# gengshan-y/ppr-diffphys

Hardware: AMD Instinct MI355X
Metric: env-steps/sec (fwd+adjoint), Laikago 12-DoF, batch=4096, 1/2/4/8 MI355X (higher is better)
Workload: dtype f32; 1 GPU; laikago, mixed mi-trot/mi-spin mocap targets, 4096 envs in total (4096 on rank 0) x 100 sim steps (4 frames), dt=5e-4, fwd+adjoint, batch split only (no collective); global_batch=4096, envs_per_gpu=4096, sim_steps=100, segment_lanes=16, nan_grads=0

## Files before the change

ppr-diffphys_amd/csrc/pd_device.h:

```cpp
#pragma once
#include "pd_math.h"

enum { PD_JOINT_REVOLUTE = 1, PD_JOINT_FIXED = 3, PD_JOINT_FREE = 4, PD_JOINT_COMPOUND = 5 };
enum { PD_JT_REVOLUTE = 1, PD_JT_COMPOUND = 2, PD_JT_FIXED = 4 };

#define PD_REC 17
#define PD_ADJ 13
#define PD_W6 7

struct PdDevModel {
  int nb, nq, nqd, nc, ntiles, max_children, max_depth;
  const int *jtype, *jparent, *qstart, *qdstart, *depth;
  const unsigned long long *children;
  const float *X_p, *X_c, *axis, *com;
  const float *lim_lo, *lim_hi, *lim_ke, *lim_kd;
  const float4 *pts;
  const unsigned char *pt_mat;
  const float4 *materials;
  const float4 *body_sphere;
  const float4 *tile_lo, *tile_hi;
  const int *tile_pack;
  const int2 *body_tiles;
  const int *small_tiles;
  unsigned long long big_bodies;
// ... 678 lines not shown
    float adj_q = 0.f;
    a_tgt[0] = 0.f; a_act[0] = 0.f; a_ke[0] = 0.f; a_kd[0] = 0.f;
    joint_force_adj(q, qd, tgt[0], ke[0], kd[0], lo, up, lke, lkd, adj_jf, adj_q, adj_qd, a_tgt[0], a_ke[0], a_kd[0], a_act[0]);
    adj_w_err += axis_p * adj_qd; adj_axis_p += j.w_err * adj_qd;
    const float adj_da = adj_q * dq_dda;
    adj_r_err.x += c.axis.x * adj_da; adj_r_err.y += c.axis.y * adj_da; adj_r_err.z += c.axis.z * adj_da;
    adj_r_err.w += adj_q * dq_dw;
    adj_qrot_q(j.q_p, c.axis, adj_q_p, adj_axis_p);
    adj_qrot_q(s.r, c.axis, adj_q_c, adj_axis_c);
  }
  if ((JT & PD_JT_COMPOUND) && (ALL || c.type == PD_JOINT_COMPOUND)) {
    const v3 ax[3] = {V3(1, 0, 0), P.ax1, P.ax2};
    v3 adj_f_raw = clamp3_pass(f_raw, adj_f, 1.0e4f);
    adj_x_err += adj_f_raw * ake; adj_v_err += adj_f_raw * akd;
    v3 adj_t_raw = clamp3_pass(P.t_raw, adj_t, 1.0e4f);
    float adj_ang[3] = {0.f, 0.f, 0.f};
    v3 adj_ax[3] = {V3(0, 0, 0), V3(0, 0, 0), V3(0, 0, 0)};
    qt adj_q_w = Q4(0, 0, 0, 0);
    const float *Mw = P.Mw;
    float aW[9];
#pragma unroll
    for (int k = 0; k < 9; ++k) aW[k] = 0.f;
#pragma unroll
    for (int k = 2; k >= 0; --k) {
      float adj_jf = dot(adj_t_raw, P.axw[k]);
      v3 adj_axw = adj_t_raw * P.jf[k];
      float adj_qdk = 0.f;
      a_tgt[k] = 0.f; a_act[k] = 0.f; a_ke[k] = 0.f; a_kd[k] = 0.f;
      const JointLimit L = c.lim[k];
      joint_force_adj(P.ang[k], P.qdk[k], tgt[k], ke[k], kd[k], L.lo, L.up, L.ke, L.kd, adj_jf, adj_ang[k], adj_qdk, a_tgt[k], a_ke[k],
                      a_kd[k], a_act[k]);
      adj_axw += j.w_err * adj_qdk; adj_w_err += P.axw[k] * adj_qdk;
      adj_ax[k] += matT_vec(Mw, adj_axw);
      add_outer(aW, adj_axw, ax[k]);
    }
    rotm_adj(P.q_w, aW, adj_q_w);
    if (HP) adj_q_p += adj_q_w; else adj_qmul_a(c.q_off, adj_q_p, adj_q_w);
    const float s0 = P.sc0.x, c0 = P.sc0.y;
    qt G;
    {
      const qt q = P.q10;
      const v3 g = adj_ax[2];
      G = Q4(g.x * (2.0f * q.z) - g.y * (2.0f * q.w), g.x * (2.0f * q.w) + g.y * (2.0f * q.z),
             g.x * (2.0f * q.x) + g.y * (2.0f * q.y) + g.z * (4.0f * q.z), g.x * (2.0f * q.y) - g.y * (2.0f * q.x) + g.z * (4.0f * q.w));
    }
    const qt adj_q_1 = Q4(c0 * G.x - s0 * G.w, c0 * G.y - s0 * G.z, c0 * G.z + s0 * G.y, c0 * G.w + s0 * G.x);
    float adj_q0x = P.q_1.w * G.x - P.q_1.y * G.z + P.q_1.z * G.y;
    float adj_q0w = P.q_1.w * G.w + P.q_1.y * G.y + P.q_1.z * G.z;
    adj_q_axis_angle_sc(ax[1], P.sc1.x, P.sc1.y, adj_ax[1], adj_ang[1], adj_q_1);
    adj_q0x += adj_ax[1].z * (2.0f * c0);
    adj_q0w += adj_ax[1].y * (4.0f * c0) + adj_ax[1].z * (2.0f * s0);
    adj_ang[0] += 0.5f * (c0 * adj_q0x - s0 * adj_q0w);
    qt adj_q_pc = Q4(0, 0, 0, 0);
    quat_decompose_adj(P.q_pc, P.c0, P.c1, P.c2, adj_ang, adj_q_pc);
    qt adj_qb = Q4(0, 0, 0, 0), adj_qa = adj_qb, adj_cqp = adj_qb;
    if (HP) adj_qb += adj_q_pc; else adj_qmul_a(c.q_off, adj_qb, adj_q_pc);
    adj_qmul(P.qa, s.r, adj_qa, adj_q_c, adj_qb);
    if (HP) adj_cqp += adj_qa; else adj_qmul_b(qconj(c.q_off), adj_cqp, adj_qa);
    adj_q_p += qconj(adj_cqp);
  }
  if (!((JT & PD_JT_COMPOUND) && (ALL || c.type == PD_JOINT_COMPOUND))) {
    qt adj_cqp = Q4(0, 0, 0, 0);
    adj_qmul(qconj(j.q_p), s.r, adj_cqp, adj_q_c, adj_r_err);
    adj_q_p += qconj(adj_cqp);
  }
  adj_qrot_q(s.r, c.com, adj_q_c, -adj_r_c);
  own.p += adj_x_err; own.r += adj_q_c; own.w += adj_w_err; own.v += adj_v_err;
  par = adj_zero();
  if (HP || c.parent >= 0) {
    v3 adj_x_p = adj_r_p - adj_x_err;
    par.p = adj_x_p - adj_r_p;
    float aP[9];
#pragma unroll
    for (int k = 0; k < 9; ++k) aP[k] = 0.f;
    add_outer(aP, -adj_r_p, c.com_par);
    add_outer(aP, adj_x_p, c.p_pj);
    rotm_adj(j.qp, aP, par.r);
    adj_qmul_a(c.q_pj, par.r, adj_q_p);
    par.w = -adj_w_err; par.v = -adj_v_err;
  }
}

#define PD_JC 23
#define PD_QPRE 22
#define PD_QGEN 3
struct RevCache {
  qt q_p, r_err;
  v3 x_p, axis_p, axis_c;
  float q, qd, jf, dq_dda, dq_dw;
};
PD_DEV void rev_cache_store(float *d, const RevCache &R) {
  d[0] = R.q_p.x; d[1] = R.q_p.y; d[2] = R.q_p.z; d[3] = R.q_p.w; d[4] = R.r_err.x; d[5] = R.r_err.y; d[6] = R.r_err.z; d[7] = R.r_err.w;
  d[8] = R.x_p.x; d[9] = R.x_p.y; d[10] = R.x_p.z;
  d[11] = R.axis_p.x; d[12] = R.axis_p.y; d[13] = R.axis_p.z; d[14] = R.axis_c.x; d[15] = R.axis_c.y; d[16] = R.axis_c.z;
  d[17] = R.q; d[18] = R.qd; d[19] = R.jf; d[20] = R.dq_dda; d[21] = R.dq_dw;
}
PD_DEV RevCache rev_cache_load(const float *d) {
  RevCache R;
  R.q_p = ld4(d); R.r_err = ld4(d + 4); R.x_p = ld3(d + 8); R.axis_p = ld3(d + 11); R.axis_c = ld3(d + 14);
  R.q = d[17]; R.qd = d[18]; R.jf = d[19]; R.dq_dda = d[20]; R.dq_dw = d[21];
  return R;
}

template <bool HP = false>
PD_DEV RevCache rev_forward(const PdDevModel &m, const BodyConst &c, qt q_c, v3 w_c, v3 pp, qt qp, v3 w_p, float tgt, float act, float ke,
                            float kd) {
  RevCache R;
  R.x_p = c.p_pj; R.q_p = c.q_pj;
  if (HP || c.parent >= 0) {
    R.x_p = pp + qrot(qp, c.p_pj);
    R.q_p = qmul(qp, c.q_pj);
  } else {
    w_p = V3(0, 0, 0);
  }
  R.r_err = qmul(qconj(R.q_p), q_c);
  R.axis_p = qrot(R.q_p, c.axis);
  R.axis_c = qrot(q_c, c.axis);
  R.q = twist_angle(dot(qvec(R.r_err), c.axis), R.r_err.w, c.alen, R.dq_dda, R.dq_dw);
  R.qd = dot(w_c - w_p, R.axis_p);
  const JointLimit L = c.lim[0];
  R.jf = joint_force(R.q, R.qd, tgt, ke, kd, act, L.lo, L.up, L.ke, L.kd);
  return R;
}

template <bool HP = false>
PD_DEV void rev_adjoint_core(const PdDevModel &m, const BodyConst &c, const BodyState &s, v3 rc_c, v3 pp, qt qp, v3 w_p, v3 v_p, v3 rc_par,
                             const RevCache &R, float tgt, float ke, float kd, v3 gc_t, v3 gc_f, v3 gp_t, v3 gp_f, BodyAdj &own, BodyAdj &par,
                             float *aR, float &a_tgt, float &a_act, float &a_ke, float &a_kd) {
  const float ake = m.attach_ke, akd = m.attach_kd, ads = 0.01f;
  v3 r_p = V3(0, 0, 0);
  if (HP || c.parent >= 0) {
    r_p = R.x_p - (pp + rc_par);
  } else {
    pp = V3(0, 0, 0); w_p = pp; v_p = pp; qp = Q4(0, 0, 0, 1);
  }
  const v3 r_c = s.p - (s.p + rc_c);
  const v3 x_err = s.p - R.x_p, v_err = s.v - v_p, w_err = s.w - w_p;
  const v3 f_total = x_err * ake + v_err * akd;
  v3 adj_t = -gc_t, adj_f = -gc_f, adj_r_c = V3(0, 0, 0), adj_r_p = V3(0, 0, 0);
  adj_cross(r_c, f_total, adj_r_c, adj_f, -gc_t);
  if (HP || c.parent >= 0) {
    adj_t += gp_t; adj_f += gp_f;
    adj_cross(r_p, f_total, adj_r_p, adj_f, gp_t);
  }
  v3 adj_x_err = adj_f * ake, adj_v_err = adj_f * akd, adj_w_err = adj_t * (akd * ads);
  qt adj_r_err = Q4(0, 0, 0, 0), adj_q_p = Q4(0, 0, 0, 0), adj_q_c = Q4(0, 0, 0, 0);
  const float adj_jf = dot(adj_t, R.axis_p);
  v3 adj_axis_p = adj_t * R.jf, adj_axis_c = V3(0, 0, 0);
  float adj_qd = -adj_jf * (akd * ads);
  adj_axis_p += adj_t * (-R.qd * (akd * ads));
  adj_cross(R.axis_p, R.axis_c, adj_axis_p, adj_axis_c, adj_t * ake);
  float adj_q = 0.f;
  a_tgt = 0.f; a_act = 0.f; a_ke = 0.f; a_kd = 0.f;
  const JointLimit L = c.lim[0];
  joint_force_adj(R.q, R.qd, tgt, ke, kd, L.lo, L.up, L.ke, L.kd, adj_jf, adj_q, adj_qd, a_tgt, a_ke, a_kd, a_act);
  adj_w_err += R.axis_p * adj_qd; adj_axis_p += w_err * adj_qd;
  const float adj_da = adj_q * R.dq_dda;
  adj_r_err.x += c.axis.x * adj_da; adj_r_err.y += c.axis.y * adj_da; adj_r_err.z += c.axis.z * adj_da;
  adj_r_err.w += adj_q * R.dq_dw;
  adj_qrot_q(R.q_p, c.axis, adj_q_p, adj_axis_p);
  add_outer(aR, adj_axis_c, c.axis);
  {
    qt adj_cqp = Q4(0, 0, 0, 0);
    adj_qmul(qconj(R.q_p), s.r, adj_cqp, adj_q_c, adj_r_err);
    adj_q_p += qconj(adj_cqp);
  }
// ... 130 lines not shown
```

ppr-diffphys_amd/csrc/pd_kernels.hip:

```cpp
#include "pd_device.h"
#include "pd_args.h"
#include "pd_se3.h"
#include "pd_quad.h"

#if PD_POLICY == 1
#define k_rollout_fwd k_rollout_fwd_literal
#define k_rollout_bwd k_rollout_bwd_literal
#define k_rollout_bwd3 k_rollout_bwd3_literal
#define PD_LAUNCH_NAME(w) PD_CAT(PD_CAT(pd_launch_seg, w), _literal)
#define PD_SET_LDS_NAME(w) PD_CAT(PD_CAT(pd_set_lds_seg, w), _literal)
#else
#define PD_LAUNCH_NAME(w) PD_CAT(pd_launch_seg, w)
#define PD_SET_LDS_NAME(w) PD_CAT(pd_set_lds_seg, w)
#endif

#ifdef PD_STAMPS
#define STAMP_DECL unsigned long long st_acc[16] = {0, 0, 0, 0, 0, 0, 0, 0, 0, 0, 0, 0, 0, 0, 0, 0}, st_t = pd_memtime()
#define STAMP_ARGS , unsigned long long *st_acc, unsigned long long &st_t
#define STAMP_PASS , st_acc, st_t
#define STAMP(i) do { unsigned long long t2_ = pd_memtime(); st_acc[i] += t2_ - st_t; st_t = t2_; } while (0)
#define STAMP_COUNT(i, n) do { st_acc[i] += (unsigned long long)(n); } while (0)
#define STAMP_FLUSH(a) do { if ((a).dbg && (threadIdx.x & 63) == 0) for (int i_ = 0; i_ < 16; ++i_) (a).dbg[((size_t)blockIdx.x * (blockDim.x / 64) + (threadIdx.x >> 6)) * 16 + i_] = st_acc[i_]; } while (0)
__device__ __forceinline__ unsigned long long pd_memtime() {
  unsigned long long t;
// ... 1242 lines not shown
template <int SEGW, int JT, bool QUAD = false, bool SEL = false>
__global__ __launch_bounds__(PD_BLOCK) void k_rollout_bwd(PdDevModel m, RolloutArgs a) {
  static_assert(JT == PD_JT_REVOLUTE, "the wave-specialised adjoint of revolute-only plain models: every jointed body is a revolute joint on a parent body");
  extern __shared__ __attribute__((aligned(16))) unsigned char smem[];
  constexpr int EPW = Seg<SEGW>::EPW;
  const int bw = (int)blockDim.x / (QUAD ? 192 : 128);
  const int role = (int)(threadIdx.x >> 6) / bw;
  const bool contact_wave = role != 0;
  [[maybe_unused]] const int knock_role = role;
  const int lane = threadIdx.x & 63, wave = (int)(threadIdx.x >> 6) % bw;
  const int seg = lane / SEGW, l = lane % SEGW;
  const int env = (blockIdx.x * bw + wave) * EPW + seg;
  const bool env_ok = env < a.bs;
  const int ec = env_ok ? env : 0;
  const bool is_body = env_ok && l < m.nb;
  const int b = l < m.nb ? l : m.nb - 1;
  const int nb = m.nb, N = a.bs * nb;

  SweepTables tabs;
  const int env_stride = m.env_lds_floats + 2 * m.env_lds_jc + (QUAD ? m.env_lds_rec2 : 0);
  float *scratch = lds_setup<false>(m, smem, tabs, wave * EPW + seg, env_stride);
  float4 *cull = (float4 *)scratch;
  float *rec = scratch + 4 * nb, *adjf = rec + nb * PD_REC, *cslot = adjf + nb * PD_W6, *cacc = cslot + (nb + 1) * PD_ADJ;
  int *list = (int *)(cacc + nb * PD_ADJ), *hits = list + m.list_cap;
  float *slot = (float *)(hits + PD_HIT_CAP_TILES * SEGW);
  float *jc = scratch + m.env_lds_floats;
  int *sig = (int *)(scratch - (size_t)seg * env_stride + m.env_lds_floats - 4);
  if (lane == 0 && !contact_wave) { sig[0] = 0; sig[1] = 0; sig[2] = 0; sig[3] = 0; }
  __syncthreads();
  PD_KNOCK_EXIT(false, knock_role);
  if constexpr (QUAD) {
    if (!env_ok) return;
  }

  BodyConst c = load_body_const(m, b, ec);
#pragma unroll
  for (int u = 0; u < 4; ++u) c.small_e[u] = m.small_tiles[u * 64 + (l < 64 ? l : 0)];
  if (l == 0) {
#pragma unroll
    for (int k = 0; k < PD_ADJ; ++k) cslot[nb * PD_ADJ + k] = 0.f;
  }
  int cz[4];
#pragma unroll
  for (int k = 0; k < 4; ++k) cz[k] = is_body && c.child[k] >= 0 ? c.child[k] : nb;
  const float *rec_s = rec;
  const float4 *cull_s = cull;
  auto contact_hit = [&](const float *r, float4 P, float4 mat, float *out) {
    const int pb = (int)(r - rec_s) / PD_REC;
    BodyAdj o = adj_zero();
    if constexpr (QUAD) {
      ContactPre C = contact_point_adj_pre(r, cull_s[pb], P, mat);
      contact_pre_barrier(C);
      contact_point_adj_rest(C, P, mat, ld3(adjf + pb * PD_W6), ld3(adjf + pb * PD_W6 + 3), o);
    } else {
      contact_point_adj(r, cull_s[pb], P, mat, ld3(adjf + pb * PD_W6), ld3(adjf + pb * PD_W6 + 3), o);
    }
    adj_store(out, o);
  };
  if (contact_wave) {
    STAMP_DECL;
    const bool rev = is_body && c.type == PD_JOINT_REVOLUTE;
    const size_t qd_off = (size_t)ec * m.nqd + c.qdstart;
    const float ke1 = rev ? a.target_ke[qd_off] : 0.f, kd1 = rev ? a.target_kd[qd_off] : 0.f;
    const int lq = l < PD_HITLOG - 1 ? l : PD_HITLOG - 2;
    const unsigned boff_c = (unsigned)((size_t)ec * nb + b) * 4u, boff_p = (unsigned)((size_t)ec * nb + (c.parent >= 0 ? c.parent : b)) * 4u;
    const unsigned boff_qd = (unsigned)qd_off * 4u, boff_lg = (unsigned)ec * (PD_HITLOG * 4u);
    auto load_log = [&](int step, int &cnt, int &e) {
      const int *lg = a.hitlog + (size_t)__builtin_amdgcn_readfirstlane(step > 0 ? step : 0) * a.bs * PD_HITLOG;
      cnt = __float_as_int(ldg((const float *)lg, boff_lg)); e = __float_as_int(ldg((const float *)lg + 1, boff_lg + (unsigned)lq * 4u));
    };
    auto load_ctrl = [&](int step, float &tgt, float &act) {
      const size_t o = (size_t)__builtin_amdgcn_readfirstlane(step > 0 ? step : 0) * a.bs * m.nqd;
      tgt = rev ? ldg(a.refs + o, boff_qd) : 0.f; act = rev && ptr_given<SEL>(a.torques) ? ldg(a.torques + o, boff_qd) : 0.f;
    };
    auto fetch_point = [&](int cnt, int &e, float4 &P, float4 &M) {
      if (!(env_ok && l < cnt && l < PD_HITLOG - 1)) e = 0;
      P = m.pts[e & 0xffff]; M = m.materials[(e >> 16) & 0xff];
    };
    auto load_pose = [&](int step, float4 *o) {
      const float *tj = a.ws + (size_t)__builtin_amdgcn_readfirstlane(step > 0 ? step : 0) * (PD_TRAJ_G * 4) * N;
      if (rev) {
        o[0] = ldg4(tj, boff_c * 4u); o[1] = ldg4(tj + (size_t)4 * N, boff_c * 4u);
        o[2] = ldg4(tj, boff_p * 4u); o[3] = ldg4(tj + (size_t)4 * N, boff_p * 4u); o[4] = ldg4(tj + (size_t)8 * N, boff_p * 4u);
      }
    };
    int cnt_c = 0, e_c = 0, cnt_n = 0, e_n = 0;
    float4 P_c, M_c;
    float tgt_c = 0.f, act_c = 0.f;
    float4 pose[5];
#pragma unroll
    for (int k = 0; k < 5; ++k) pose[k] = make_float4(0.f, 0.f, 0.f, 0.f);
    const int qb = lane >> 2, qc = lane & 3, bbq = qb < nb ? qb : nb - 1;
    const QLane kq = q_lane(qc);
    const int qgen_floats = m.env_lds_rec2 / PD_QGEN - PD_QPRE * 64 - m.env_lds_jc;
    float *const qgen = jc + 2 * m.env_lds_jc, *const qpre = qgen + PD_QGEN * qgen_floats;
    QBody Bq;
    float npl_c[PD_TRAJ_G];
    const unsigned boff_tjq = (unsigned)(((size_t)ec * nb + bbq) * 4 + qc) * 4u;
    auto load_planes = [&](int step, float *pl) {
      const float *tj = a.ws + (size_t)__builtin_amdgcn_readfirstlane(step > 0 ? step : 0) * (PD_TRAJ_G * 4) * N;
#pragma unroll
      for (int g = 0; g < PD_TRAJ_G; ++g) pl[g] = ldg(tj + (size_t)(4 * g) * N, boff_tjq);
    };
    auto q_pre = [&](const float *pl, int g) {
      QState s;
      const float vx = Q_BC3(pl[1]), vy = Q_BC3(pl[2]), vz = Q_BC0(pl[3]);
      const float tsh = q_dpp<PD_QP(1, 2, 3, 3)>(pl[3]);
      const float maskf = Q_BC3(pl[4]);
      s.r = pl[0];
      s.w = kq.isv ? pl[1] : 0.f; s.p = kq.isv ? pl[2] : 0.f;
      s.v = qc == 0 ? vx : (qc == 1 ? vy : (qc == 2 ? vz : 0.f));
      const float t0 = kq.isv ? tsh : 0.f, f0 = kq.isv ? pl[4] : 0.f;
      QM3 Rr, Rc;
      q_rotm(kq, s.r, Rr, Rc);
      const float rc = q_mvc(Rr, Bq.com0, Bq.com1, Bq.com2);
      {
        float *G = qgen + g * qgen_floats, *r = G + 4 * nb + bbq * PD_REC;
        r[3 + qc] = s.r;
        r[kq.isv ? qc : 16] = s.p; r[kq.isv ? 7 + qc : 16] = s.w; r[kq.isv ? 10 + qc : 16] = s.v; r[kq.isv ? 13 + qc : 16] = rc;
        if (qc == 1) ((float4 *)G)[bbq] = make_float4(s.p, Rr.a, Rr.b, Rr.c);
      }
      QIntTmp T;
      q_integrate_adj_pre(kq, Bq, s, Rr, Rc, t0, a.dt, T);
      float *P = qpre + g * (PD_QPRE * 64) + lane;
      P[0 * 64] = s.p; P[1 * 64] = s.r; P[2 * 64] = s.w; P[3 * 64] = s.v; P[4 * 64] = t0; P[5 * 64] = f0; P[6 * 64] = maskf; P[7 * 64] = rc;
      P[8 * 64] = Rr.a; P[9 * 64] = Rr.b; P[10 * 64] = Rr.c; P[11 * 64] = Rc.a; P[12 * 64] = Rc.b; P[13 * 64] = Rc.c;
      P[14 * 64] = T.wb; P[15 * 64] = T.Iwb; P[16 * 64] = T.tb; P[17 * 64] = T.u; P[18 * 64] = T.w1; P[19 * 64] = T.il; P[20 * 64] = T.r1;
    };
    int g3 = a.nsteps > 0 ? (a.nsteps - 1) % PD_QGEN : 0;
    if constexpr (QUAD) {
      if (role == 2) {
        const BodyConst cb = load_body_const(m, bbq, ec);
        const size_t qidx = (size_t)ec * nb + bbq;
        const int qv = qc < 3 ? qc : 2;
        Bq.com0 = cb.com.x; Bq.com1 = cb.com.y; Bq.com2 = cb.com.z;
        const float *Ib = a.inertia + qidx * 9, *Jb = a.inv_inertia + qidx * 9;
        Bq.I.a = kq.isv ? Ib[qv * 3] : 0.f; Bq.I.b = kq.isv ? Ib[qv * 3 + 1] : 0.f; Bq.I.c = kq.isv ? Ib[qv * 3 + 2] : 0.f;
        Bq.invI.a = kq.isv ? Jb[qv * 3] : 0.f; Bq.invI.b = kq.isv ? Jb[qv * 3 + 1] : 0.f; Bq.invI.c = kq.isv ? Jb[qv * 3 + 2] : 0.f;
        float *const jcq = qpre + PD_QGEN * (PD_QPRE * 64);
        if (a.nsteps > 0) { load_ctrl(a.nsteps - 1, tgt_c, act_c); load_pose(a.nsteps - 1, pose); load_planes(a.nsteps - 1, npl_c); }
        for (int step = a.nsteps - 1; step >= 0; --step) {
          PD_WAIT_VMEM();
          pair_wait(sig, a.nsteps - step - (PD_QGEN - 1));
          if (rev) {
            const qt q_c = Q4(pose[0].x, pose[0].y, pose[0].z, pose[0].w), qp = Q4(pose[2].x, pose[2].y, pose[2].z, pose[2].w);
            const v3 w_c = V3(pose[1].x, pose[1].y, pose[1].z), pp = V3(pose[4].x, pose[4].y, pose[4].z), w_p = V3(pose[3].x, pose[3].y, pose[3].z);
            rev_cache_store(jcq + g3 * m.env_lds_jc + b * PD_JC, rev_forward<true>(m, c, q_c, w_c, pp, qp, w_p, tgt_c, act_c, ke1, kd1));
          }
          q_pre(npl_c, g3);
          load_ctrl(step - 1, tgt_c, act_c); load_pose(step - 1, pose); load_planes(step - 1, npl_c);
          pair_signal(sig + 1, a.nsteps - step);
          g3 = g3 == 0 ? PD_QGEN - 1 : g3 - 1;
        }
        return;
      }
    }
    if (a.nsteps > 0) {
      load_log(a.nsteps - 1, cnt_c, e_c);
      if constexpr (!QUAD) { load_ctrl(a.nsteps - 1, tgt_c, act_c); load_pose(a.nsteps - 1, pose); }
      load_log(a.nsteps - 2, cnt_n, e_n);
      fetch_point(cnt_c, e_c, P_c, M_c);
    }
    for (int step = a.nsteps - 1; step >= 0; --step) {
      PD_WAIT_VMEM();
      if (!QUAD && rev)
      {
        const qt q_c = Q4(pose[0].x, pose[0].y, pose[0].z, pose[0].w), qp = Q4(pose[2].x, pose[2].y, pose[2].z, pose[2].w);
        const v3 w_c = V3(pose[1].x, pose[1].y, pose[1].z), pp = V3(pose[4].x, pose[4].y, pose[4].z), w_p = V3(pose[3].x, pose[3].y, pose[3].z);
        float *dst = jc + (step & 1) * m.env_lds_jc + b * PD_JC;
        rev_cache_store(dst, rev_forward<true>(m, c, q_c, w_c, pp, qp, w_p, tgt_c, act_c, ke1, kd1));
      }
      STAMP(8);
      float tgt_n, act_n;
      float4 P_n, M_n;
      int cnt_n2, e_n2;
      fetch_point(cnt_n, e_n, P_n, M_n);
      if constexpr (!QUAD) {
        load_ctrl(step - 1, tgt_n, act_n);
        load_pose(step - 1, pose);
      } else {
        tgt_n = 0.f; act_n = 0.f;
      }
      load_log(step - 2, cnt_n2, e_n2);
      const bool fast = __ballot(env_ok && (cnt_c < 0 || cnt_c > SEGW)) == 0ull;
      const int nh = fast && env_ok ? cnt_c : 0;
      STAMP(7);
      if constexpr (!QUAD) pair_signal(sig + 1, a.nsteps - step);
      const int pb = l < nh ? (e_c >> 24) & 0x3f : -2;
      ContactPre cpre;
      cpre.touch = false;
      if constexpr (QUAD) {
        pair_wait(sig + 1, a.nsteps - step);
        rec_s = qgen + g3 * qgen_floats + 4 * nb;
        cull_s = (const float4 *)(qgen + g3 * qgen_floats);
        if (fast && l < nh) cpre = contact_point_adj_pre(rec_s + pb * PD_REC, cull_s[pb], P_c, M_c);
      }
      pair_wait(sig, a.nsteps - step);
      __builtin_amdgcn_s_setprio(PD_PRIO_CRITICAL);
      STAMP(9);
      if (fast) {
        float out[PD_ADJ];
#pragma unroll
        for (int i = 0; i < PD_ADJ; ++i) out[i] = 0.f;
        if constexpr (QUAD) {
          if (l < nh) {
            BodyAdj o = adj_zero();
            contact_pre_barrier(cpre);
            contact_point_adj_rest(cpre, P_c, M_c, ld3(adjf + pb * PD_W6), ld3(adjf + pb * PD_W6 + 3), o);
            adj_store(out, o);
          }
        } else {
          if (l < nh) contact_hit(rec_s + pb * PD_REC, P_c, M_c, out);
        }
        STAMP(10);
        bool last;
        seg_run_sum<PD_ADJ>(out, pb, l, nh, last);
        if (last) {
#pragma unroll
          for (int i = 0; i < PD_ADJ; ++i) cacc[pb * PD_ADJ + i] = out[i];
        }
        STAMP(11);
      } else {
        float4 cv = make_float4(0.f, 0.f, 1.f, 0.f);
        if (is_body) cv = cull_s[b];
        int *lg = a.hitlog + ((size_t)step * a.bs + ec) * PD_HITLOG;
        const bool replay = __ballot(env_ok && cnt_c < 0) == 0ull;
        int log_n_unused;
        sweep_contacts<SEGW, PD_ADJ, PD_ADJ, false>(m, tabs, c, cv, rec_s, cull_s, list, hits, slot, cacc, is_body, env_ok, seg, l,
                                                    replay ? lg : nullptr, replay ? (env_ok ? cnt_c : 0) : PD_NO_REPLAY, log_n_unused,
                                                    contact_hit STAMP_PASS);
      }
      STAMP(12);
      pair_signal(sig + 2, a.nsteps - step);
      __builtin_amdgcn_s_setprio(0);
      cnt_c = cnt_n; e_c = e_n; P_c = P_n; M_c = M_n; tgt_c = tgt_n; act_c = act_n;
      cnt_n = cnt_n2; e_n = e_n2;
      if constexpr (QUAD) g3 = g3 == 0 ? PD_QGEN - 1 : g3 - 1;
    }
    STAMP_FLUSH(a);
    return;
  }
  if constexpr (QUAD) {
    static_assert(SEGW == 64, "quad-lane body wave: one env per wave");
    const int qb = lane >> 2, qc = lane & 3, bb = qb < nb ? qb : nb - 1, qv = qc < 3 ? qc : 2;
    const bool qbody = true;
    float *const dummy = adjf + bb * PD_W6 + 6;
    const QLane k = q_lane(qc);
    const size_t qidx = (size_t)ec * nb + bb;
    QBody B;
    QM3 It, invIt;
    float com_par0, com_par1, com_par2, p_pj0, p_pj1, p_pj2;
    QPerm pjc;
    {
      const BodyConst cb = load_body_const(m, bb, ec);
      B.type = cb.type; B.pidx = cb.pidx; B.qdstart = cb.qdstart;
      B.joint = qbody && cb.type == PD_JOINT_REVOLUTE;
      B.com = q_pick(k, cb.com); B.com0 = cb.com.x; B.com1 = cb.com.y; B.com2 = cb.com.z;
      B.axis = q_pick(k, cb.axis); B.ax0 = cb.axis.x; B.ax1 = cb.axis.y; B.ax2 = cb.axis.z; B.alen = cb.alen;
      B.p_pj = q_pick(k, cb.p_pj); B.q_pj = q_pick(k, cb.q_pj); B.pj = q_perm(k, B.q_pj);
      pjc = q_perm(k, B.q_pj * k.sc);
      com_par0 = cb.com_par.x; com_par1 = cb.com_par.y; com_par2 = cb.com_par.z;
      p_pj0 = cb.p_pj.x; p_pj1 = cb.p_pj.y; p_pj2 = cb.p_pj.z;
      B.g = q_pick(k, V3(m.gx, m.gy, m.gz));
      B.reach = cb.reach; B.sphere_w = cb.sphere.w; B.lim = cb.lim[0];
      B.inv_m = a.inv_mass[qidx];
      const bool on = cb.type == PD_JOINT_REVOLUTE;
      B.ke = on ? a.target_ke[(size_t)ec * m.nqd + cb.qdstart] : 0.f;
      B.kd = on ? a.target_kd[(size_t)ec * m.nqd + cb.qdstart] : 0.f;
      const float *Ib = a.inertia + qidx * 9, *Jb = a.inv_inertia + qidx * 9;
      B.I.a = k.isv ? Ib[qv * 3] : 0.f; B.I.b = k.isv ? Ib[qv * 3 + 1] : 0.f; B.I.c = k.isv ? Ib[qv * 3 + 2] : 0.f;
      B.invI.a = k.isv ? Jb[qv * 3] : 0.f; B.invI.b = k.isv ? Jb[qv * 3 + 1] : 0.f; B.invI.c = k.isv ? Jb[qv * 3 + 2] : 0.f;
      It.a = k.isv ? Ib[qv] : 0.f; It.b = k.isv ? Ib[3 + qv] : 0.f; It.c = k.isv ? Ib[6 + qv] : 0.f;
      invIt.a = k.isv ? Jb[qv] : 0.f; invIt.b = k.isv ? Jb[3 + qv] : 0.f; invIt.c = k.isv ? Jb[6 + qv] : 0.f;
    }
    int qcz[4];
    const unsigned long long q_children = m.children[bb];
#pragma unroll
    for (int j = 0; j < 4; ++j) { const int cid = (int)((q_children >> (8 * j)) & 0xffull); qcz[j] = (qbody && cid != 0xff) ? cid : nb; }
    if (lane < PD_ADJ) cslot[nb * PD_ADJ + lane] = 0.f;
    float *const ca_r = cacc + bb * PD_ADJ + 3 + qc, *const ca_p = k.isv ? cacc + bb * PD_ADJ + qc : dummy,
                *const ca_w = k.isv ? cacc + bb * PD_ADJ + 7 + qc : dummy, *const ca_v = k.isv ? cacc + bb * PD_ADJ + 10 + qc : dummy;
    float *const cs_r = cslot + bb * PD_ADJ + 3 + qc, *const cs_p = k.isv ? cslot + bb * PD_ADJ + qc : dummy,
                *const cs_w = k.isv ? cslot + bb * PD_ADJ + 7 + qc : dummy, *const cs_v = k.isv ? cslot + bb * PD_ADJ + 10 + qc : dummy;
    *ca_r = 0.f; *ca_p = 0.f; *ca_w = 0.f; *ca_v = 0.f;
    QM3 g_I, g_invI;
    g_I.a = g_I.b = g_I.c = 0.f; g_invI = g_I;
    float g_inv_m = 0.f, g_ke = 0.f, g_kd = 0.f;
    QAdj gn;
    gn.p = gn.r = gn.w = gn.v = 0.f;
    const unsigned boff_tj = (unsigned)(qidx * 4 + qc) * 4u, boff_qd = (unsigned)((size_t)ec * m.nqd + B.qdstart) * 4u;
    const unsigned boff_rf = (unsigned)(qidx * 6 + qv) * 4u;
    float n_tgt = 0.f;
    int n_fr = -1;
    auto load_step = [&](int step) {
      const int sc = __builtin_amdgcn_readfirstlane(step >= 0 ? step : 0);
      n_fr = a.frame_of_step[sc + 1];
      const size_t o = (size_t)sc * a.bs * m.nqd;
      n_tgt = ldg(a.refs + o, boff_qd);
    };
    const float ake = m.attach_ke, akd = m.attach_kd;
    const int qgen_floats = m.env_lds_rec2 / PD_QGEN - PD_QPRE * 64 - m.env_lds_jc;
    float *const qgen = jc + 2 * m.env_lds_jc, *const qpre = qgen + PD_QGEN * qgen_floats;
    QState s;
    float t0 = 0.f, f0 = 0.f, tgt = 0.f, rc = 0.f, sd_p = 0.f, sd_r = 0.f, sd_w = 0.f, sd_v = 0.f;
    unsigned mask = 0u;
    QM3 Rr, Rc;
    QIntTmp T;
    auto q_ahead = [&](int step) {
      const int fr = n_fr;
      sd_p = 0.f; sd_r = 0.f; sd_w = 0.f; sd_v = 0.f;
      if (fr >= 0) {
        const float *gp = a.adj_pos + ((size_t)fr * N + qidx) * 7, *gv = a.adj_vel + ((size_t)fr * N + qidx) * 6;
        sd_p = gp[qv]; sd_r = gp[3 + qc]; sd_w = gv[qv]; sd_v = gv[3 + qv];
      }
      tgt = n_tgt;
      load_step(step - 1);
    };
    auto q_take = [&](int g) {
      const float *P = qpre + g * (PD_QPRE * 64) + lane;
      s.p = P[0 * 64]; s.r = P[1 * 64]; s.w = P[2 * 64]; s.v = P[3 * 64]; t0 = P[4 * 64]; f0 = P[5 * 64]; mask = __float_as_uint(P[6 * 64]); rc = P[7 * 64];
// ... 112 lines not shown
    auto q_seeds = [&](int fr) {
      const float *gp = a.adj_pos + ((size_t)fr * N + qidx) * 7, *gv = a.adj_vel + ((size_t)fr * N + qidx) * 6;
      const float sp = gp[qv], sr = gp[3 + qc], sw = gv[qv], sv = gv[3 + qv];
      gn.p += k.isv ? sp : 0.f; gn.r += sr; gn.w += k.isv ? sw : 0.f; gn.v += k.isv ? sv : 0.f;
    };
    if (a.frame_of_step[0] >= 0) q_seeds(a.frame_of_step[0]);
    float *const rec0 = qgen + 4 * nb;
    WAVE_SYNC();
    if (qbody) {
      float *d = a.g_state0 ? a.g_state0 + qidx * PD_ADJ : cacc + bb * PD_ADJ;
      d[3 + qc] = gn.r;
      if (k.isv) { d[qc] = gn.p; d[7 + qc] = gn.w; d[10 + qc] = gn.v; }
    }
    WAVE_SYNC();
    if (!a.g_state0) {
      BodyAdj gs = adj_zero();
      if (is_body) adj_add_from(gs, cacc + b * PD_ADJ);
      if (a.nsteps == 0) {
        for (int d = 0; d <= m.max_depth; ++d) {
          if (is_body && c.depth == d) {
            BodyState s0 = fk_joint<JT>(c, a.q_init + (size_t)ec * m.nq + c.qstart, a.qd_init + (size_t)ec * m.nqd + c.qdstart, rec0);
            stage_record(rec0, b, s0, c.com);
          }
          WAVE_SYNC();
        }
      }
      for (int d = m.max_depth; d >= 0; --d) {
        if (is_body && c.depth == d) {
          for (int j = 0; j < m.max_children; ++j) {
            int cid = (int)((c.children >> (8 * j)) & 0xffull);
            if (cid != 0xff) adj_add_from(gs, cslot + cid * PD_ADJ);
          }
          BodyAdj pr_ = fk_joint_adj<JT, 1>(c, a.q_init + (size_t)ec * m.nq + c.qstart, a.qd_init + (size_t)ec * m.nqd + c.qdstart, rec0,
                                          gs, a.g_q_init + (size_t)ec * m.nq + c.qstart, a.g_qd_init + (size_t)ec * m.nqd + c.qdstart);
          adj_store(cslot + b * PD_ADJ, pr_);
        }
        WAVE_SYNC();
      }
    }
    if (qbody) {
      if (qc == 0) a.g_inv_mass[qidx] = NZ(g_inv_m);
      if (k.isv) {
        float *gi = a.g_inertia + qidx * 9 + qc * 3, *gj = a.g_inv_inertia + qidx * 9 + qc * 3;
        gi[0] = NZ(g_I.a); gi[1] = NZ(g_I.b); gi[2] = NZ(g_I.c);
        gj[0] = NZ(g_invI.a); gj[1] = NZ(g_invI.b); gj[2] = NZ(g_invI.c);
      }
      const size_t og = (size_t)ec * m.nqd + B.qdstart;
      if (B.type == PD_JOINT_REVOLUTE && qc == 0) { a.g_ke[og] = NZ(g_ke); a.g_kd[og] = NZ(g_kd); }
      if (B.type == PD_JOINT_FREE) {
        a.g_ke[og + qc] = 0.f; a.g_kd[og + qc] = 0.f;
        if (qc < 2) { a.g_ke[og + 4 + qc] = 0.f; a.g_kd[og + 4 + qc] = 0.f; }
      }
    }
    return;
  }
  constexpr int ND = 1;
  const size_t idx = (size_t)ec * nb + b;
  const int ndof = c.type == PD_JOINT_REVOLUTE ? 1 : (c.type == PD_JOINT_COMPOUND ? 3 : 0);

  float inv_m = a.inv_mass[idx], I[9], invI[9], ke[ND], kd[ND];
#pragma unroll
  for (int k = 0; k < 9; ++k) { I[k] = a.inertia[idx * 9 + k]; invI[k] = a.inv_inertia[idx * 9 + k]; }
#pragma unroll
  for (int k = 0; k < ND; ++k) {
    bool on = k < ndof;
    ke[k] = on ? a.target_ke[(size_t)ec * m.nqd + c.qdstart + k] : 0.f;
    kd[k] = on ? a.target_kd[(size_t)ec * m.nqd + c.qdstart + k] : 0.f;
  }
  float g_inv_m = 0.f, g_I[9], g_invI[9], g_ke[ND], g_kd[ND];
#pragma unroll
  for (int k = 0; k < 9; ++k) { g_I[k] = 0.f; g_invI[k] = 0.f; }
#pragma unroll
  for (int k = 0; k < ND; ++k) { g_ke[k] = 0.f; g_kd[k] = 0.f; }
  if (is_body) {
#pragma unroll
    for (int k = 0; k < PD_ADJ; ++k) cacc[b * PD_ADJ + k] = 0.f;
  }

  BodyAdj gn = adj_zero();
  BodyState s;
  s.p = V3(0, 0, 0); s.r = Q4(0, 0, 0, 1); s.w = V3(0, 0, 0); s.v = V3(0, 0, 0);

  const unsigned boff = (unsigned)idx * 4u, boff_qd = (unsigned)((size_t)ec * m.nqd + c.qdstart) * 4u;
  const bool zero_by_lanes = m.jtype[0] == PD_JOINT_FREE && nb >= 7;
  const unsigned boff_zero = (unsigned)((size_t)ec * m.nqd + m.qdstart[0] + (b >= 1 && b <= 6 ? b - 1 : 0)) * 4u;
  float4 n_s[PD_TRAJ_G];
  float n_tgt[ND];
  int n_fr = -1;
  auto load_step = [&](int step) {
    const int sc = __builtin_amdgcn_readfirstlane(step >= 0 ? step : 0);
    n_fr = a.frame_of_step[sc + 1];
    const float *tj = a.ws + (size_t)sc * (PD_TRAJ_G * 4) * N;
#pragma unroll
    for (int g = 0; g < PD_TRAJ_G; ++g) n_s[g] = ldg4(tj + (size_t)(4 * g) * N, boff * 4u);
    const size_t o = (size_t)sc * a.bs * m.nqd;
#pragma unroll
    for (int k = 0; k < ND; ++k) {
      bool on = k < ndof;
      n_tgt[k] = on ? ldg(a.refs + o + k, boff_qd) : 0.f;
    }
  };
  if (a.nsteps > 0) load_step(a.nsteps - 1);
  STAMP_DECL;
  for (int step = a.nsteps - 1; step >= 0; --step) {
    PD_WAIT_VMEM();
    {
      const int fr = n_fr;
      if (fr >= 0) {
        add_frame_seeds(a, fr, N, idx, gn);
      }
    }
    s.r = Q4(n_s[0].x, n_s[0].y, n_s[0].z, n_s[0].w); s.w = V3(n_s[1].x, n_s[1].y, n_s[1].z);
    s.p = V3(n_s[2].x, n_s[2].y, n_s[2].z); s.v = V3(n_s[1].w, n_s[2].w, n_s[3].x);
    v3 t0 = V3(n_s[3].y, n_s[3].z, n_s[3].w), f0 = V3(n_s[4].x, n_s[4].y, n_s[4].z);
    const unsigned clamp_mask = __float_as_uint(n_s[4].w);
    float tgt[ND];
#pragma unroll
    for (int k = 0; k < ND; ++k) tgt[k] = n_tgt[k];
    const size_t oc = (size_t)step * a.bs * m.nqd;
    load_step(step - 1);
    float Rm[9];
    rotm(s.r, Rm);
    const v3 rc = mat_vec(Rm, c.com);
    if (is_body) stage_record(rec, cull, b, s, rc, Rm);
    STAMP(0);
    BodyAdj ga = adj_zero();
    v3 adj_t0 = V3(0, 0, 0), adj_f0 = adj_t0;
    float aR[9];
#pragma unroll
    for (int k = 0; k < 9; ++k) aR[k] = 0.f;
    integrate_adj(m, c, s, Rm, clamp_mask, t0, f0, inv_m, I, invI, a.dt, gn, ga, aR, adj_t0, adj_f0, g_inv_m, g_I, g_invI);
    if (is_body) {
      float *f = adjf + b * PD_W6;
      f[0] = adj_t0.x; f[1] = adj_t0.y; f[2] = adj_t0.z; f[3] = adj_f0.x; f[4] = adj_f0.y; f[5] = adj_f0.z;
    }
    STAMP(1);
    pair_signal(sig, a.nsteps - step);
    if (grad_wanted<SEL>(a.g_res_f) && is_body) {
      float *o = a.g_res_f + (size_t)step * N * 6;
      stg2(o, boff * 6u, make_float2(NZ(adj_t0.x), NZ(adj_t0.y))); stg2(o + 2, boff * 6u, make_float2(NZ(adj_t0.z), NZ(adj_f0.x)));
      stg2(o + 4, boff * 6u, make_float2(NZ(adj_f0.y), NZ(adj_f0.z)));
    }
    pair_wait(sig + 1, a.nsteps - step);
    BodyAdj par = adj_zero();
    float a_tgt[ND], a_act[ND], a_ke[ND], a_kd[ND];
#pragma unroll
    for (int k = 0; k < ND; ++k) { a_tgt[k] = 0.f; a_act[k] = 0.f; a_ke[k] = 0.f; a_kd[k] = 0.f; }
    if (is_body && c.type != PD_JOINT_FREE) {
      const v3 gp_t = ld3(adjf + c.parent * PD_W6), gp_f = ld3(adjf + c.parent * PD_W6 + 3);
      const RevCache R = rev_cache_load(jc + (step & 1) * m.env_lds_jc + b * PD_JC);
      rev_adjoint<true>(m, c, s, rc, rec, R, tgt[0], ke[0], kd[0], adj_t0, adj_f0, gp_t, gp_f, ga, par, aR, a_tgt[0], a_act[0], a_ke[0], a_kd[0]);
    }
    rotm_adj(s.r, aR, ga.r);
    if (is_body) {
      adj_store(cslot + b * PD_ADJ, par);
#pragma unroll
      for (int k = 0; k < ND; ++k) {
        if (k < ndof) {
          if (grad_wanted<SEL>(a.g_refs)) stg(a.g_refs + oc + k, boff_qd, NZ(a_tgt[k]));
          if (grad_wanted<SEL>(a.g_torques)) stg(a.g_torques + oc + k, boff_qd, NZ(a_act[k]));
        }
        g_ke[k] += a_ke[k]; g_kd[k] += a_kd[k];
      }
      if (zero_by_lanes) {
        if (b >= 1 && b <= 6) {
          if (grad_wanted<SEL>(a.g_refs)) stg(a.g_refs + oc, boff_zero, 0.f);
          if (grad_wanted<SEL>(a.g_torques)) stg(a.g_torques + oc, boff_zero, 0.f);
        }
      } else if (c.type == PD_JOINT_FREE) {
#pragma unroll
        for (int k = 0; k < 6; ++k) {
          if (grad_wanted<SEL>(a.g_refs)) stg(a.g_refs + oc + k, boff_qd, 0.f);
          if (grad_wanted<SEL>(a.g_torques)) stg(a.g_torques + oc + k, boff_qd, 0.f);
        }
      }
    }
    STAMP(2);
    WAVE_SYNC();
    {
      const float *const src[4] = {cslot + cz[0] * PD_ADJ, cslot + cz[1] * PD_ADJ, cslot + cz[2] * PD_ADJ, cslot + cz[3] * PD_ADJ};
      adj_add_from_n(ga, src);
    }
    for (int k = 4; k < m.max_children; ++k) {
      int cid = (int)((c.children >> (8 * k)) & 0xffull);
      if (is_body && cid != 0xff) adj_add_from(ga, cslot + cid * PD_ADJ);
    }
    STAMP(3);
    pair_wait(sig + 2, a.nsteps - step);
    if (is_body) {
      float *d = cacc + b * PD_ADJ;
      const float *const src[1] = {d};
      adj_add_from_n(ga, src);
#pragma unroll
      for (int k = 0; k < PD_ADJ; ++k) d[k] = 0.f;
    }
    gn = ga;
    STAMP(4);
  }
  STAMP_FLUSH(a);
  {
    int fr = a.frame_of_step[0];
    if (fr >= 0) {
      add_frame_seeds(a, fr, N, idx, gn);
    }
  }
  if (a.g_state0 && is_body) adj_store(a.g_state0 + idx * PD_ADJ, gn);
  const int fk_levels = a.g_state0 ? -1 : m.max_depth;
  if (a.nsteps == 0) {
    for (int d = 0; d <= fk_levels; ++d) {
      if (is_body && c.depth == d) {
        s = fk_joint<JT>(c, a.q_init + (size_t)ec * m.nq + c.qstart, a.qd_init + (size_t)ec * m.nqd + c.qdstart, rec);
        stage_record(rec, b, s, c.com);
      }
      WAVE_SYNC();
    }
  }
  for (int d = fk_levels; d >= 0; --d) {
    if (is_body && c.depth == d) {
      for (int k = 0; k < m.max_children; ++k) {
        int cid = (int)((c.children >> (8 * k)) & 0xffull);
        if (cid != 0xff) adj_add_from(gn, cslot + cid * PD_ADJ);
      }
      BodyAdj par = fk_joint_adj<JT, 1>(c, a.q_init + (size_t)ec * m.nq + c.qstart, a.qd_init + (size_t)ec * m.nqd + c.qdstart, rec,
                                     gn, a.g_q_init + (size_t)ec * m.nq + c.qstart, a.g_qd_init + (size_t)ec * m.nqd + c.qdstart);
      adj_store(cslot + b * PD_ADJ, par);
    }
    WAVE_SYNC();
  }
  if (is_body) {
    a.g_inv_mass[idx] = NZ(g_inv_m);
#pragma unroll
    for (int k = 0; k < 9; ++k) { a.g_inertia[idx * 9 + k] = NZ(g_I[k]); a.g_inv_inertia[idx * 9 + k] = NZ(g_invI[k]); }
    const size_t og = (size_t)ec * m.nqd + c.qdstart;
#pragma unroll
    for (int k = 0; k < ND; ++k)
      if (k < ndof) { a.g_ke[og + k] = NZ(g_ke[k]); a.g_kd[og + k] = NZ(g_kd[k]); }
    if (c.type == PD_JOINT_FREE) {
#pragma unroll
      for (int k = 0; k < 6; ++k) { a.g_ke[og + k] = 0.f; a.g_kd[og + k] = 0.f; }
    }
  }
}

template <int SEGW, int JT, bool GT = false, bool SEL = false>
__global__ __launch_bounds__(PD_BLOCK) void k_rollout_bwd3(PdDevModel m, RolloutArgs a) {
  extern __shared__ __attribute__((aligned(16))) unsigned char smem[];
  constexpr int EPW = Seg<SEGW>::EPW;
  constexpr int ND = (JT & PD_JT_COMPOUND) ? 3 : 1;
  static_assert(JT != PD_JT_REVOLUTE, "revolute-only models take k_rollout_bwd");
  const int bw = (int)blockDim.x / (64 * 2);
  const int lane = threadIdx.x & 63, wave_id = threadIdx.x >> 6;
  const int role = wave_id / bw ? 2 : 0, wave = wave_id % bw;
  [[maybe_unused]] const int knock_role = role;
  const int seg = lane / SEGW, l = lane % SEGW;
  const int env = (blockIdx.x * bw + wave) * EPW + seg;
  const bool env_ok = env < a.bs;
  const int ec = env_ok ? env : 0;
  const bool is_body = env_ok && l < m.nb;
  const int b = l < m.nb ? l : m.nb - 1;
  const int nb = m.nb, N = a.bs * nb;

  SweepTables tabs;
  float *scratch = lds_setup<!GT>(m, smem, tabs, wave * EPW + seg, m.env_lds_bwd3);
  float4 *const cull0 = (float4 *)scratch;
  float *const rec0 = scratch + 8 * nb;
  float4 *cull = cull0;
  float *rec = rec0;
  auto select_step = [&](int step) { rec = rec0 + (step & 1) * nb * PD_REC; cull = cull0 + (step & 1) * nb; };
  float *adjf = rec0 + 2 * nb * PD_REC, *cslot = adjf + nb * PD_W6, *oslot = cslot + (nb + 1) * PD_ADJ;
  float *cacc = oslot + nb * PD_ADJ;
  float *gacc = cacc + nb * PD_ADJ;
  int *list = (int *)(gacc + (nb + 1) * PD_GACC), *hits = list + m.list_cap;
  float *slot = (float *)(hits + PD_HIT_CAP_TILES * SEGW);
  int *sig = (int *)(scratch - (size_t)seg * m.env_lds_bwd3 + m.env_lds_bwd3 - 4);
  if (role == 0) {
    if (lane == 0) { sig[0] = 0; sig[1] = 0; sig[2] = 0; sig[3] = 0; }
    if (is_body) {
#pragma unroll
      for (int k = 0; k < PD_ADJ; ++k) { cacc[b * PD_ADJ + k] = 0.f; oslot[b * PD_ADJ + k] = 0.f; cslot[b * PD_ADJ + k] = 0.f; }
    }
    if (l == 0) {
// ... 528 lines not shown
```

Before: 909.5 million env-steps/s.

## Offload adjoint gradient global stores from the critical wave to its contact partner wave

The paired-wave backward kernel moves the global stores of residual-force gradients and per-step reference and torque gradients out of the dynamics wave's critical loop. The dynamics wave now stashes the control gradients in two spare slots of the joint cache in LDS, and the contact wave reads them and issues the stores after releasing its priority. This takes store issue off the serial adjoint chain. In exchange it adds a one-step delay with an extra final signal and wait to flush step 0, plus more LDS traffic and a dependency on slot lifetimes in the double-buffered joint cache.

Measured after the change: 881.2 million env-steps/s. 3.1% lower.

```diff
diff --git a/ppr-diffphys_amd/csrc/pd_device.h b/ppr-diffphys_amd/csrc/pd_device.h
--- a/ppr-diffphys_amd/csrc/pd_device.h
+++ b/ppr-diffphys_amd/csrc/pd_device.h
@@ -784,6 +784,8 @@
 }
 
 #define PD_JC 23
+#define PD_JC_GT 21
+#define PD_JC_GA 22
 #define PD_QPRE 22
 #define PD_QGEN 3
 struct RevCache {
diff --git a/ppr-diffphys_amd/csrc/pd_kernels.hip b/ppr-diffphys_amd/csrc/pd_kernels.hip
--- a/ppr-diffphys_amd/csrc/pd_kernels.hip
+++ b/ppr-diffphys_amd/csrc/pd_kernels.hip
@@ -1348,6 +1348,20 @@
       if (rev) {
         o[0] = ldg4(tj, boff_c * 4u); o[1] = ldg4(tj + (size_t)4 * N, boff_c * 4u);
         o[2] = ldg4(tj, boff_p * 4u); o[3] = ldg4(tj + (size_t)4 * N, boff_p * 4u); o[4] = ldg4(tj + (size_t)8 * N, boff_p * 4u);
+      }
+    };
+    [[maybe_unused]] const bool zero_by_lanes = m.jtype[0] == PD_JOINT_FREE && nb >= 7;
+    [[maybe_unused]] const unsigned boff_zero = (unsigned)((size_t)ec * m.nqd + m.qdstart[0] + (b >= 1 && b <= 6 ? b - 1 : 0)) * 4u;
+    [[maybe_unused]] const bool ctrl_wanted = grad_wanted<SEL>(a.g_refs) || grad_wanted<SEL>(a.g_torques);
+    [[maybe_unused]] auto take_ctrl = [&](int step, float &gt, float &ga) {
+      const float *h = jc + (step & 1) * m.env_lds_jc + b * PD_JC;
+      gt = h[PD_JC_GT]; ga = h[PD_JC_GA];
+    };
+    [[maybe_unused]] auto store_ctrl = [&](int step, float gt, float ga) {
+      const size_t oc = (size_t)__builtin_amdgcn_readfirstlane(step) * a.bs * m.nqd;
+      if (rev) {
+        if (grad_wanted<SEL>(a.g_refs)) stg(a.g_refs + oc, boff_qd, NZ(gt));
+        if (grad_wanted<SEL>(a.g_torques)) stg(a.g_torques + oc, boff_qd, NZ(ga));
       }
     };
     int cnt_c = 0, e_c = 0, cnt_n = 0, e_n = 0;
@@ -1464,6 +1478,14 @@
       pair_wait(sig, a.nsteps - step);
       __builtin_amdgcn_s_setprio(PD_PRIO_CRITICAL);
       STAMP(9);
+      [[maybe_unused]] float rf[6], gt_p = 0.f, ga_p = 0.f;
+      if constexpr (!QUAD) {
+        if (grad_wanted<SEL>(a.g_res_f)) {
+#pragma unroll
+          for (int k = 0; k < 6; ++k) rf[k] = adjf[b * PD_W6 + k];
+        }
+        if (ctrl_wanted) take_ctrl(step + 1, gt_p, ga_p);
+      }
       if (fast) {
         float out[PD_ADJ];
 #pragma unroll
@@ -1499,9 +1521,40 @@
       STAMP(12);
       pair_signal(sig + 2, a.nsteps - step);
       __builtin_amdgcn_s_setprio(0);
+      if constexpr (!QUAD) {
+        if (grad_wanted<SEL>(a.g_res_f) && is_body) {
+          float *o = a.g_res_f + (size_t)__builtin_amdgcn_readfirstlane(step) * N * 6;
+          stg2(o, boff_c * 6u, make_float2(NZ(rf[0]), NZ(rf[1]))); stg2(o + 2, boff_c * 6u, make_float2(NZ(rf[2]), NZ(rf[3])));
+          stg2(o + 4, boff_c * 6u, make_float2(NZ(rf[4]), NZ(rf[5])));
+        }
+        if (ctrl_wanted) {
+          if (step + 1 < a.nsteps) store_ctrl(step + 1, gt_p, ga_p);
+          const size_t oc = (size_t)__builtin_amdgcn_readfirstlane(step) * a.bs * m.nqd;
+          if (zero_by_lanes) {
+            if (is_body && b >= 1 && b <= 6) {
+              if (grad_wanted<SEL>(a.g_refs)) stg(a.g_refs + oc, boff_zero, 0.f);
+              if (grad_wanted<SEL>(a.g_torques)) stg(a.g_torques + oc, boff_zero, 0.f);
+            }
+          } else if (is_body && c.type == PD_JOINT_FREE) {
+#pragma unroll
+            for (int k = 0; k < 6; ++k) {
+              if (grad_wanted<SEL>(a.g_refs)) stg(a.g_refs + oc + k, boff_qd, 0.f);
+              if (grad_wanted<SEL>(a.g_torques)) stg(a.g_torques + oc + k, boff_qd, 0.f);
+            }
+          }
+        }
+      }
       cnt_c = cnt_n; e_c = e_n; P_c = P_n; M_c = M_n; tgt_c = tgt_n; act_c = act_n;
       cnt_n = cnt_n2; e_n = e_n2;
       if constexpr (QUAD) g3 = g3 == 0 ? PD_QGEN - 1 : g3 - 1;
+    }
+    if constexpr (!QUAD) {
+      if (ctrl_wanted && a.nsteps > 0) {
+        float gt_p, ga_p;
+        pair_wait(sig, a.nsteps + 1);
+        take_ctrl(0, gt_p, ga_p);
+        store_ctrl(0, gt_p, ga_p);
+      }
     }
     STAMP_FLUSH(a);
     return;
@@ -1780,8 +1833,6 @@
   s.p = V3(0, 0, 0); s.r = Q4(0, 0, 0, 1); s.w = V3(0, 0, 0); s.v = V3(0, 0, 0);
 
   const unsigned boff = (unsigned)idx * 4u, boff_qd = (unsigned)((size_t)ec * m.nqd + c.qdstart) * 4u;
-  const bool zero_by_lanes = m.jtype[0] == PD_JOINT_FREE && nb >= 7;
-  const unsigned boff_zero = (unsigned)((size_t)ec * m.nqd + m.qdstart[0] + (b >= 1 && b <= 6 ? b - 1 : 0)) * 4u;
   float4 n_s[PD_TRAJ_G];
   float n_tgt[ND];
   int n_fr = -1;
@@ -1815,7 +1866,6 @@
     float tgt[ND];
 #pragma unroll
     for (int k = 0; k < ND; ++k) tgt[k] = n_tgt[k];
-    const size_t oc = (size_t)step * a.bs * m.nqd;
     load_step(step - 1);
     float Rm[9];
     rotm(s.r, Rm);
@@ -1834,11 +1884,6 @@
     }
     STAMP(1);
     pair_signal(sig, a.nsteps - step);
-    if (grad_wanted<SEL>(a.g_res_f) && is_body) {
-      float *o = a.g_res_f + (size_t)step * N * 6;
-      stg2(o, boff * 6u, make_float2(NZ(adj_t0.x), NZ(adj_t0.y))); stg2(o + 2, boff * 6u, make_float2(NZ(adj_t0.z), NZ(adj_f0.x)));
-      stg2(o + 4, boff * 6u, make_float2(NZ(adj_f0.y), NZ(adj_f0.z)));
-    }
     pair_wait(sig + 1, a.nsteps - step);
     BodyAdj par = adj_zero();
     float a_tgt[ND], a_act[ND], a_ke[ND], a_kd[ND];
@@ -1846,32 +1891,16 @@
     for (int k = 0; k < ND; ++k) { a_tgt[k] = 0.f; a_act[k] = 0.f; a_ke[k] = 0.f; a_kd[k] = 0.f; }
     if (is_body && c.type != PD_JOINT_FREE) {
       const v3 gp_t = ld3(adjf + c.parent * PD_W6), gp_f = ld3(adjf + c.parent * PD_W6 + 3);
-      const RevCache R = rev_cache_load(jc + (step & 1) * m.env_lds_jc + b * PD_JC);
+      float *const h = jc + (step & 1) * m.env_lds_jc + b * PD_JC;
+      const RevCache R = rev_cache_load(h);
       rev_adjoint<true>(m, c, s, rc, rec, R, tgt[0], ke[0], kd[0], adj_t0, adj_f0, gp_t, gp_f, ga, par, aR, a_tgt[0], a_act[0], a_ke[0], a_kd[0]);
+      h[PD_JC_GT] = a_tgt[0]; h[PD_JC_GA] = a_act[0];
     }
     rotm_adj(s.r, aR, ga.r);
     if (is_body) {
       adj_store(cslot + b * PD_ADJ, par);
 #pragma unroll
-      for (int k = 0; k < ND; ++k) {
-        if (k < ndof) {
-          if (grad_wanted<SEL>(a.g_refs)) stg(a.g_refs + oc + k, boff_qd, NZ(a_tgt[k]));
-          if (grad_wanted<SEL>(a.g_torques)) stg(a.g_torques + oc + k, boff_qd, NZ(a_act[k]));
-        }
-        g_ke[k] += a_ke[k]; g_kd[k] += a_kd[k];
-      }
-      if (zero_by_lanes) {
-        if (b >= 1 && b <= 6) {
-          if (grad_wanted<SEL>(a.g_refs)) stg(a.g_refs + oc, boff_zero, 0.f);
-          if (grad_wanted<SEL>(a.g_torques)) stg(a.g_torques + oc, boff_zero, 0.f);
-        }
-      } else if (c.type == PD_JOINT_FREE) {
-#pragma unroll
-        for (int k = 0; k < 6; ++k) {
-          if (grad_wanted<SEL>(a.g_refs)) stg(a.g_refs + oc + k, boff_qd, 0.f);
-          if (grad_wanted<SEL>(a.g_torques)) stg(a.g_torques + oc + k, boff_qd, 0.f);
-        }
-      }
+      for (int k = 0; k < ND; ++k) { g_ke[k] += a_ke[k]; g_kd[k] += a_kd[k]; }
     }
     STAMP(2);
     WAVE_SYNC();
@@ -1895,6 +1924,7 @@
     gn = ga;
     STAMP(4);
   }
+  if (a.nsteps > 0) pair_signal(sig, a.nsteps + 1);
   STAMP_FLUSH(a);
   {
     int fr = a.frame_of_step[0];
```
